# faircloth-lab/tapir

Hardware: AMD Instinct MI355X
Metric: alignment columns/sec (site-rate+PI) (higher is better)
Workload: dtype f64

## Files before the change

tapir_amd/csrc/launch_constants.hpp:

```cpp
#pragma once
#include <cstddef>
#include <cstdint>

namespace tphip {

constexpr int kFirstStepMinTaxa = 32;
constexpr int kSiteBlock = 64;
constexpr int kReserveShift = 16;
constexpr int kShareWeightShift = 10;
constexpr double kDefaultReserve = 0.15;
constexpr int kTailFillsBig = 5, kTailFillsMid = 3, kTailFillsSmall = 2;
constexpr double kTailFracBig = 0.4, kTailFracMid = 0.3;
constexpr int kMixedLoci = 8;
constexpr int kMixedLdsHeader = kMixedLoci * 64 + 64 + 32;
constexpr int kMixedColBits = 28;
constexpr int kSiteLdsHeader = 160;
constexpr int kStreamWords = -1;
constexpr int kStreamWordsSpill = -2;
constexpr int kMixedVariant = 100;

#ifndef TPHIP_LIK_BLOCK
#define TPHIP_LIK_BLOCK 128
#endif
constexpr int kLikBlock = TPHIP_LIK_BLOCK;
constexpr int kGradBlock = 128;
constexpr int kGradWaves = kGradBlock / 64;
constexpr int kGradEF = 12;
constexpr int kGradSlots = 4;
constexpr size_t kValueWorkspaceBytes = (size_t)1 << 30;
constexpr int kValueTipRow = 20;
constexpr int kValueMaxDepth = 5;
constexpr int kGrad2Block = 128;
constexpr int kGrad2Waves = kGrad2Block / 64;
constexpr int kGrad2EF = 12;
constexpr int kGrad2MaxRDepth = 8;

constexpr int kPiBlock = 256;
constexpr int kPiColsPerThread = 4;
constexpr int kPiChunk = kPiBlock * kPiColsPerThread;

enum : int32_t { DEDUP_AUTO = 0, DEDUP_OFF = 1, DEDUP_ON = 2 };
constexpr int64_t kDedupAutoMinColumns = 1 << 20;

}
```

tapir_amd/csrc/pi_kernels.hpp:

```cpp
#pragma once
#include <hip/hip_runtime.h>
#include <cstdint>
#include "gtr_model.hpp"
#include "tree_program.hpp"
#include "quadpack_device.hpp"
#include "site_rate_params.hpp"
#include "pi_rate.hpp"
#include "tphip.h"
#include "wave_sum.hpp"

namespace tphip {

constexpr int kTimeTile = 16;
constexpr int kIvTile = 8;

struct ClassifyParams {
    const uint8_t* states;
    int64_t ncols_total;
    int32_t ntaxa;
    const LocusModel* models;
    const int64_t* locus_offsets;
    const int32_t* chunk_locus;
    const int32_t* chunk_index;
    double* rate;
    double* subst;
    double* lnl;
    uint8_t* flag;
    int32_t* nres;
    double chrono_length;
    const int2* steps;
    int32_t tail_pops;
    int32_t max_pops;
    uint32_t* packed;
    double start_scale;
    uint64_t* hash;
};

typedef const __attribute__((address_space(4))) int2 ConstInt2;
__device__ __forceinline__ ConstInt2* as_constant(const int2* p) { return (ConstInt2*)(uintptr_t)p; }

struct ColumnScan {
    unsigned uni = 0;
    int resolved = 0, informative = 0;
    unsigned changes = 0;
    int base[3] = {0, 0, 0};
};

struct ColumnScan4 {
    static constexpr uint32_t k01 = 0x01010101u, k0f = 0x0f0f0f0fu;
    uint32_t uni4 = 0, set4 = k0f;
    uint32_t res8 = 0, inf8 = 0, chg8 = 0;
    uint32_t a8 = 0, c8 = 0, g8 = 0;
    int base[3][4] = {{0, 0, 0, 0}, {0, 0, 0, 0}, {0, 0, 0, 0}};
    uint64_t hsh[4] = {0x243F6A8885A308D3ull, 0x243F6A8885A308D3ull, 0x243F6A8885A308D3ull, 0x243F6A8885A308D3ull};
    int resolved[4] = {0, 0, 0, 0}, informative[4] = {0, 0, 0, 0};
    unsigned changes[4] = {0, 0, 0, 0};
    unsigned long long stk[4] = {0, 0, 0, 0};
    static __device__ __forceinline__ uint32_t nonzero(uint32_t x) { return ((x + k0f) >> 4) & k01; }
    static __device__ __forceinline__ uint32_t is15(uint32_t x) { return ((x + k01) >> 4) & k01; }
    static __device__ __forceinline__ uint32_t spread(uint32_t b) {
        uint32_t s = b << 4;
        asm("" : "+v"(s));
        return s - b;
    }
    __device__ __forceinline__ void flush() {
#pragma unroll
        for (int j = 0; j < 4; ++j) {
            resolved[j] += (int)((res8 >> (8 * j)) & 0xffu);
            informative[j] += (int)((inf8 >> (8 * j)) & 0xffu);
            changes[j] += (chg8 >> (8 * j)) & 0xffu;
            base[0][j] += (int)((a8 >> (8 * j)) & 0xffu);
            base[1][j] += (int)((c8 >> (8 * j)) & 0xffu);
            base[2][j] += (int)((g8 >> (8 * j)) & 0xffu);
        }
        res8 = inf8 = chg8 = 0;
        a8 = c8 = g8 = 0;
    }
    __device__ __forceinline__ void fitch_join(uint32_t x4) {
        const uint32_t both = set4 & x4;
        const uint32_t empty = nonzero(both) ^ k01;
        chg8 += empty;
        set4 = both | ((set4 | x4) & spread(empty));
    }
    __device__ __forceinline__ void fitch_push() {
#pragma unroll
        for (int j = 0; j < 4; ++j) stk[j] = (stk[j] << 4) | ((set4 >> (8 * j)) & 15u);
        set4 = k0f;
    }
    __device__ __forceinline__ void fitch_pop() {
        uint32_t x4 = 0;
#pragma unroll
        for (int j = 0; j < 4; ++j) { x4 |= (uint32_t)(stk[j] & 15ull) << (8 * j); stk[j] >>= 4; }
        fitch_join(x4);
    }
    __device__ __forceinline__ uint32_t tip(uint32_t v) {
        uint32_t m4 = v & k0f;
        m4 |= spread(nonzero(m4) ^ k01);
        const uint32_t res = is15(m4) ^ k01;
        uni4 |= m4 & spread(res);
        res8 += res;
        const uint32_t single = nonzero(m4 & (m4 - k01)) ^ k01;
        inf8 += single;
        a8 += single & m4;
        c8 += single & (m4 >> 1);
        g8 += single & (m4 >> 2);
        fitch_join(m4);
        return m4;
    }
    static __device__ __forceinline__ void pack8(const uint32_t* m, uint32_t* word) {
        const uint32_t a01 = m[0] | (m[1] << 4), a23 = m[2] | (m[3] << 4), a45 = m[4] | (m[5] << 4), a67 = m[6] | (m[7] << 4);
        const uint32_t t_lo = __builtin_amdgcn_perm(a23, a01, 0x05010400u);
        const uint32_t t_hi = __builtin_amdgcn_perm(a23, a01, 0x07030602u);
        const uint32_t u_lo = __builtin_amdgcn_perm(a67, a45, 0x05010400u);
        const uint32_t u_hi = __builtin_amdgcn_perm(a67, a45, 0x07030602u);
        word[0] = __builtin_amdgcn_perm(u_lo, t_lo, 0x05040100u);
        word[1] = __builtin_amdgcn_perm(u_lo, t_lo, 0x07060302u);
        word[2] = __builtin_amdgcn_perm(u_hi, t_hi, 0x05040100u);
        word[3] = __builtin_amdgcn_perm(u_hi, t_hi, 0x07060302u);
    }
    __device__ __forceinline__ ColumnScan column(int j) const {
        ColumnScan c;
        c.uni = (uni4 >> (8 * j)) & 15u;
        c.resolved = resolved[j];
        c.informative = informative[j];
        c.changes = changes[j];
        c.base[0] = base[0][j]; c.base[1] = base[1][j]; c.base[2] = base[2][j];
// ... 112 lines not shown
            for (int j = 0; j < 4; ++j) {
                uint64_t h = (c.hsh[j] ^ word[j]) * 0x9E3779B97F4A7C15ull;
                c.hsh[j] = h ^ (h >> 29);
            }
        }
    };
    const int ngroups = (P.ntaxa + 7) >> 3;
    uint32_t b0[8], b1[8];
    load_group(0, b0);
    int g = 0;
    for (; g + 1 < ngroups; g += 2) {
        load_group(g + 1, b1);
        asm volatile("" ::: "memory");
        group(g, b0);
        if (g + 2 < ngroups) load_group(g + 2, b0);
        asm volatile("" ::: "memory");
        group(g + 1, b1);
    }
    if (g < ngroups) group(g, b0);
    for (int q = P.tail_pops; q > 0; --q) c.fitch_pop();
}

__global__ __launch_bounds__(kPiBlock) void classify_kernel(ClassifyParams P) {
    const int locus = P.chunk_locus[blockIdx.x];
    const int64_t lo = P.locus_offsets[locus], hi = P.locus_offsets[locus + 1];
    const LocusModel* __restrict__ M = P.models + locus;
    const int64_t c0 = lo + (int64_t)P.chunk_index[blockIdx.x] * kPiChunk + 4 * (int64_t)threadIdx.x;
    if (c0 >= hi) return;
    const bool full = (c0 + 4 <= hi);
    const bool aligned = full && ((reinterpret_cast<uintptr_t>(P.states) & 3u) == 0) && ((P.ncols_total & 3) == 0) &&
                         ((c0 & 3) == 0);
    const int n = full ? 4 : (int)(hi - c0);
    const bool fast = __all(aligned);
    ColumnScan4 c;
    if (fast) {
        if (P.max_pops <= kMaxUnrolledPops) classify_scan<true, true>(P, c0, n, c);
        else classify_scan<true, false>(P, c0, n, c);
    } else {
        classify_scan<false, false>(P, c0, n, c);
    }
    c.flush();
    uint8_t f[4] = {0, 0, 0, 0};
    double ex[4];
    exit_rates(M, ex);
#pragma unroll
    for (int j = 0; j < 4; ++j) if (j < n) classify_finish(P, M, c0 + j, c.column(j), ex, f[j]);
    if (P.hash) {
#pragma unroll
        for (int j = 0; j < 4; ++j) if (j < n) P.hash[c0 + j] = c.hsh[j] ^ (c.hsh[j] >> 32);
    }
    if (fast) {
        *reinterpret_cast<int4*>(P.nres + c0) = make_int4(c.informative[0], c.informative[1], c.informative[2], c.informative[3]);
        *reinterpret_cast<uint32_t*>(P.flag + c0) = (uint32_t)f[0] | ((uint32_t)f[1] << 8) | ((uint32_t)f[2] << 16) | ((uint32_t)f[3] << 24);
    } else {
#pragma unroll
        for (int j = 0; j < 4; ++j) {
            if (j < n) { P.nres[c0 + j] = c.informative[j]; P.flag[c0 + j] = f[j]; }
        }
    }
}

template <int kCompactBlock>
__global__ __launch_bounds__(kCompactBlock) void compact_kernel(const uint8_t* __restrict__ flag, const int64_t* __restrict__ locus_offsets,
                                                                int32_t* __restrict__ work_cols, int32_t* __restrict__ work_count) {
    constexpr int kWaves = kCompactBlock / 64;
    __shared__ int wave_tot[kWaves];
    __shared__ int running;
// ... 436 lines not shown
        double r[kPiColsPerThread];
        bool ok[kPiColsPerThread];
        pi_pack_chunk(P, base, hi, packed_rate, r, ok);
#pragma unroll
        for (int j = 0; j < kPiColsPerThread; ++j) n_ok += ok[j] ? 1 : 0;
    }
    double* out = P.partial + (size_t)chunk * (P.T + 2 * P.n_i);
    for (int k0 = 0; k0 < P.n_i; k0 += kIvSplitTile) {
        int a[kIvSplitTile], b[kIvSplitTile];
#pragma unroll
        for (int kk = 0; kk < kIvSplitTile; ++kk) {
            const int k = (k0 + kk < P.n_i) ? k0 + kk : P.n_i - 1;
            a[kk] = __builtin_amdgcn_readfirstlane(P.intervals[2 * k]);
            b[kk] = __builtin_amdgcn_readfirstlane(P.intervals[2 * k + 1]);
        }
        double si[kIvSplitTile], se[kIvSplitTile];
#pragma unroll
        for (int kk = 0; kk < kIvSplitTile; ++kk) { si[kk] = 0.0; se[kk] = 0.0; }
#pragma unroll 1
        for (int j = 0; j < n_ok; ++j) {
            const double rj = packed_rate[j * kPiBlock + (int)threadIdx.x];
            GkFactors F;
            double have_h = -1.0;
#pragma unroll
            for (int kk = 0; kk < kIvSplitTile; ++kk) {
                if (k0 + kk < P.n_i) {
                    int ai = a[kk], bi = b[kk];
                    asm volatile("" : "+s"(ai), "+s"(bi));
                    const double aj = (double)ai, bj = (double)bi;
                    double res, err = 0.0;
                    if (P.integ_mode == TPHIP_INTEG_QUADPACK) {
                        const double hl = 0.5 * (bj - aj);
                        if (4.0 * rj * hl < 30.0) {
                            if (hl != have_h) { gk_factors(rj, hl, F); have_h = hl; }
                            quad_townsend_factored(aj, bj, rj, F, res, err);
                        } else {
                            const QuadResult g = quad_townsend_generic(aj, bj, rj);
                            res = g.result;
                            err = g.abserr;
                        }
                    } else {
                        res = integral_closed(aj, bj, rj);
                    }
                    si[kk] += res;
                    se[kk] += err;
                }
            }
        }
#pragma unroll
        for (int kk = 0; kk < kIvSplitTile; ++kk) {
            if (k0 + kk < P.n_i) {
                const double s1 = wave_sum(si[kk]), s2 = wave_sum(se[kk]);
                if (lane == 0) { red[2 * kk][wave] = s1; red[2 * kk + 1][wave] = s2; }
            }
        }
        __syncthreads();
        if (threadIdx.x < 2 * kIvSplitTile && k0 + (int)(threadIdx.x >> 1) < P.n_i) {
            const int kk = threadIdx.x >> 1, which = threadIdx.x & 1;
            out[P.T + which * P.n_i + k0 + kk] =
                ((red[threadIdx.x][0] + red[threadIdx.x][1]) + red[threadIdx.x][2]) + red[threadIdx.x][3];
        }
        __syncthreads();
    }
}

constexpr int kPiReduceBlock = 64;
__global__ __launch_bounds__(kPiReduceBlock) void pi_reduce_kernel(const double* __restrict__ partial, const int64_t* __restrict__ locus_chunk_offsets,
                                 int32_t T, const int32_t* __restrict__ times, int32_t n_t, int32_t n_i,
// ... 82 lines not shown
```

tapir_amd/csrc/quadpack_device.hpp:

```cpp
#pragma once
#include <hip/hip_runtime.h>
#include <cfloat>
#include "fast_exp.hpp"

namespace tphip {

template <bool TAB>
__device__ __forceinline__ double townsend_pi(double t, double r, const double* __restrict__ etab) {
#pragma clang fp contract(off)
    const double x = -(4.0 * r * t);
    if constexpr (TAB) return 16.0 * (r * r) * t * exp_nonpos_tab(fmin(x, 0.0), etab);
    else return 16.0 * (r * r) * t * exp(x);
}

struct GK21 {
    double result, abserr, resabs, resasc;
};

__device__ __constant__ const double kXgk[11] = {
    0.995657163025808080735527280689003, 0.973906528517171720077964012084452, 0.930157491355708226001207180059508,
    0.865063366688984510732096688423493, 0.780817726586416897063717578345042, 0.679409568299024406234327365114874,
    0.562757134668604683339000099272694, 0.433395394129247190799265943165784, 0.294392862701460198131126603103866,
    0.148874338981631210884826001129720, 0.0};
__device__ __constant__ const double kWgk[11] = {
    0.011694638867371874278064396062192, 0.032558162307964727478818972459390, 0.054755896574351996031381300244580,
    0.075039674810919952767043140916190, 0.093125454583697605535065465083366, 0.109387158802297641899210590325805,
    0.123491976262065851077958109585166, 0.134709217311473325928054001771707, 0.142775938577060080797094273138717,
    0.147739104901338491374841515972068, 0.149445554002916905664936468389821};
__device__ __constant__ const double kWg[5] = {
    0.066671344308688137593568809893332, 0.149451349150580593145776339657697, 0.219086362515982043995534934228163,
    0.269266719309996355091226921569469, 0.295524224714752870173815619188769};

template <bool TAB>
__device__ __forceinline__ GK21 dqk21(double rate, double a, double b, const double* __restrict__ etab) {
#pragma clang fp contract(off)
    const double epmach = DBL_EPSILON, uflow = DBL_MIN;
    double fv1[10], fv2[10];
    const double centr = 0.5 * (a + b), hlgth = 0.5 * (b - a), dhlgth = fabs(hlgth);
    double resg = 0.0;
    const double fc = townsend_pi<TAB>(centr, rate, etab);
    double resk = kWgk[10] * fc;
    double resabs = fabs(resk);
#pragma unroll
    for (int j = 0; j < 5; ++j) {
        const int jtw = 2 * j + 1;
        const double absc = hlgth * kXgk[jtw];
        const double f1 = townsend_pi<TAB>(centr - absc, rate, etab), f2 = townsend_pi<TAB>(centr + absc, rate, etab);
        fv1[jtw] = f1; fv2[jtw] = f2;
        const double fsum = f1 + f2;
        resg += kWg[j] * fsum;
        resk += kWgk[jtw] * fsum;
        resabs += kWgk[jtw] * (fabs(f1) + fabs(f2));
    }
#pragma unroll
    for (int j = 0; j < 5; ++j) {
        const int jtwm1 = 2 * j;
        const double absc = hlgth * kXgk[jtwm1];
        const double f1 = townsend_pi<TAB>(centr - absc, rate, etab), f2 = townsend_pi<TAB>(centr + absc, rate, etab);
        fv1[jtwm1] = f1; fv2[jtwm1] = f2;
        const double fsum = f1 + f2;
        resk += kWgk[jtwm1] * fsum;
        resabs += kWgk[jtwm1] * (fabs(f1) + fabs(f2));
    }
    const double reskh = resk * 0.5;
    double resasc = kWgk[10] * fabs(fc - reskh);
#pragma unroll
    for (int j = 0; j < 10; ++j) resasc += kWgk[j] * (fabs(fv1[j] - reskh) + fabs(fv2[j] - reskh));
    GK21 o;
    o.result = resk * hlgth;
    o.resabs = resabs * dhlgth;
    o.resasc = resasc * dhlgth;
    double abserr = fabs((resk - resg) * hlgth);
    if (o.resasc != 0.0 && abserr != 0.0) {
        const double q = 200.0 * abserr / o.resasc;
        const double q15 = q * sqrt(q);
        abserr = o.resasc * fmin(1.0, q15);
    }
    if (o.resabs > uflow / (50.0 * epmach)) abserr = fmax((epmach * 50.0) * o.resabs, abserr);
    o.abserr = abserr;
    return o;
}

struct GkFactors {
    double fm[10];
    double fp[10];
};

__device__ __forceinline__ void gk_factors(double rate, double hlgth, GkFactors& F) {
#pragma clang fp contract(off)
#pragma unroll
    for (int j = 0; j < 10; ++j) {
        const double absc = hlgth * kXgk[j];
        F.fm[j] = exp(-(4.0 * rate * absc));
        F.fp[j] = 1.0 / F.fm[j];
    }
}

__device__ __forceinline__ GK21 dqk21_factored(double rate, double a, double b, const GkFactors& F) {
#pragma clang fp contract(off)
    const double epmach = DBL_EPSILON, uflow = DBL_MIN;
    double fv1[10], fv2[10];
    const double centr = 0.5 * (a + b), hlgth = 0.5 * (b - a), dhlgth = fabs(hlgth);
    const double c16 = 16.0 * (rate * rate);
    const double ec = exp(-(4.0 * rate * centr));
    double resg = 0.0;
    const double fc = c16 * centr * ec;
    double resk = kWgk[10] * fc;
    double resabs = fabs(resk);
#pragma unroll
    for (int j = 0; j < 5; ++j) {
        const int jtw = 2 * j + 1;
        const double absc = hlgth * kXgk[jtw];
        const double f1 = c16 * (centr - absc) * (ec * F.fp[jtw]), f2 = c16 * (centr + absc) * (ec * F.fm[jtw]);
        fv1[jtw] = f1; fv2[jtw] = f2;
        const double fsum = f1 + f2;
        resg += kWg[j] * fsum;
        resk += kWgk[jtw] * fsum;
        resabs += kWgk[jtw] * (fabs(f1) + fabs(f2));
    }
#pragma unroll
    for (int j = 0; j < 5; ++j) {
        const int jtwm1 = 2 * j;
        const double absc = hlgth * kXgk[jtwm1];
        const double f1 = c16 * (centr - absc) * (ec * F.fp[jtwm1]), f2 = c16 * (centr + absc) * (ec * F.fm[jtwm1]);
        fv1[jtwm1] = f1; fv2[jtwm1] = f2;
        const double fsum = f1 + f2;
        resk += kWgk[jtwm1] * fsum;
        resabs += kWgk[jtwm1] * (fabs(f1) + fabs(f2));
    }
    const double reskh = resk * 0.5;
    double resasc = kWgk[10] * fabs(fc - reskh);
#pragma unroll
    for (int j = 0; j < 10; ++j) resasc += kWgk[j] * (fabs(fv1[j] - reskh) + fabs(fv2[j] - reskh));
    GK21 o;
    o.result = resk * hlgth;
    o.resabs = resabs * dhlgth;
    o.resasc = resasc * dhlgth;
    double abserr = fabs((resk - resg) * hlgth);
    if (o.resasc != 0.0 && abserr != 0.0) {
        const double q = 200.0 * abserr / o.resasc;
        const double q15 = q * sqrt(q);
        abserr = o.resasc * fmin(1.0, q15);
    }
    if (o.resabs > uflow / (50.0 * epmach)) abserr = fmax((epmach * 50.0) * o.resabs, abserr);
    o.abserr = abserr;
    return o;
}

__device__ inline void dqpsrt(int limit, int last, int* maxerr, double* ermax, const double* elist, int* iord, int* nrmax) {
    if (last <= 2) {
        iord[1] = 1; iord[2] = 2;
    } else {
        const double errmax = elist[*maxerr];
        if (*nrmax != 1) {
            const int ido = *nrmax - 1;
            for (int i = 1; i <= ido; ++i) {
                const int isucc = iord[*nrmax - 1];
                if (errmax <= elist[isucc]) break;
                iord[*nrmax] = isucc;
                --*nrmax;
            }
        }
        int jupbn = last;
        if (last > (limit / 2 + 2)) jupbn = limit + 3 - last;
        const double errmin = elist[last];
        const int jbnd = jupbn - 1;
// ... 195 lines not shown
            if (ierro == 3) abserr += correc;
            if (ier == 0) ier = 3;
            if (result != 0.0 && area != 0.0) {
                if (abserr / fabs(result) > errsum / fabs(area)) sum_lists = true;
            } else if (abserr > errsum) {
                sum_lists = true;
            }
        }
        (void)ksgn;
    }
    if (sum_lists) {
        result = 0.0;
        for (int k = 1; k <= last; ++k) result += rlist[k];
        abserr = errsum;
    }
    *result_out = result;
    *abserr_out = abserr;
}

template <bool TAB>
__device__ __forceinline__ void quad_townsend(double a, double b, double rate, const double* __restrict__ etab, double& result,
                                              double& abserr) {
#pragma clang fp contract(off)
    const double epsabs = 1.49e-8, epsrel = 1.49e-8, epmach = DBL_EPSILON;
    const GK21 g = dqk21<TAB>(rate, a, b, etab);
    result = g.result;
    abserr = g.abserr;
    const double errbnd = fmax(epsabs, epsrel * fabs(g.result));
    const bool roundoff = (g.abserr <= 100.0 * epmach * g.resabs && g.abserr > errbnd);
    const bool accept = roundoff || (g.abserr <= errbnd && g.abserr != g.resasc) || g.abserr == 0.0;
    if (!accept) dqagse_adaptive<TAB>(rate, a, b, g, etab, &result, &abserr);
}

__device__ __forceinline__ void quad_townsend_factored(double a, double b, double rate, const GkFactors& F, double& result,
                                                       double& abserr) {
#pragma clang fp contract(off)
    const double epsabs = 1.49e-8, epsrel = 1.49e-8, epmach = DBL_EPSILON;
    const GK21 g = dqk21_factored(rate, a, b, F);
    result = g.result;
    abserr = g.abserr;
    const double errbnd = fmax(epsabs, epsrel * fabs(g.result));
    const bool roundoff = (g.abserr <= 100.0 * epmach * g.resabs && g.abserr > errbnd);
    const bool accept = roundoff || (g.abserr <= errbnd && g.abserr != g.resasc) || g.abserr == 0.0;
    if (!accept) dqagse_adaptive<false>(rate, a, b, g, nullptr, &result, &abserr);
}

__device__ __forceinline__ double integral_closed(double a, double b, double r) {
    const double xa = 4.0 * r * a, d = 4.0 * r * (b - a);
    double m = 0.0, g = 0.0;
    if (d < 0.1) {
        double term = d;
        for (int k = 1; k < 40; ++k) {
            const double add = term * (double)(k - 1);
            m += (k & 1) ? term : -term;
            g += (k & 1) ? -add : add;
            if (k > 1 && add <= 1e-20 * fabs(g)) break;
            term = term * d / (double)(k + 1);
        }
    } else {
        const double e = exp(-d);
        m = 1.0 - e;
        g = m - d * e;
    }
    return exp(-xa) * (xa * m + g);
}

}
```

tapir_amd/csrc/site_driver.hip:

```cpp
#include <hip/hip_runtime.h>

#include <cstdio>
#include <cstdlib>

#include "dedup_kernels.hpp"
#include "pi_kernels.hpp"
#include "tphip_internal.hpp"

extern "C" {

int tphip_profile_enable(tphip_plan* p, int32_t on) {
    if (!p) return fail(TPHIP_ERR_INVALID, "null plan");
    HIP_TRY(hipSetDevice(p->device));
    if (on && p->ev.empty()) {
        p->ev.resize(4 * kProfileRing);
        for (auto& e : p->ev) HIP_TRY(hipEventCreate(&e));
    }
    p->profile = on != 0;
    return TPHIP_OK;
}

static int profile_drain(tphip_plan* p) {
    for (int s = 0; s < p->ev_used; ++s) {
        float ms = 0;
// ... 29 lines not shown
        for (tphip_plan* q : p->parts) {
            HIP_TRY(hipMemcpy(&w, q->d_evals.p + which, sizeof w, hipMemcpyDeviceToHost));
            v += w;
        }
    } else {
        HIP_TRY(hipMemcpy(&v, p->d_evals.p + which, sizeof v, hipMemcpyDeviceToHost));
    }
    *out = (int64_t)v;
    return TPHIP_OK;
}

int tphip_last_eval_count(tphip_plan* p, int64_t* evals) {
    const int rc = last_count(p, 0, evals);
    if (rc == TPHIP_OK && !p->last_run_in_parts && getenv("TPHIP_SITE_TRACE_ROUNDS")) {
        unsigned long long c[8];
        HIP_TRY(hipMemcpy(c, p->d_evals.p, sizeof c, hipMemcpyDeviceToHost));
        if (c[5]) fprintf(stderr, "site_rate_kernel: %llu waves with work, evaluations %llu, rounds mean %.1f max %llu (lane use %.1f %%), wave time mean %.1f us max %.1f us\n",
                          c[5], c[0], (double)c[1] / c[5], c[2], 100.0 * c[0] / (64.0 * c[1]), 0.01 * c[3] / c[5], 0.01 * c[4]);
    }
    return rc;
}

int tphip_last_round_count(tphip_plan* p, int64_t* rounds) { return last_count(p, 1, rounds); }


static ClassifyParams classify_params(const tphip_plan* p, const uint8_t* d_states, double* rate, double* subst, double* lnl, uint8_t* flag,
                                      int32_t* nres, uint32_t* packed, uint64_t* hash, double start_scale) {
    ClassifyParams C{};
    C.states = d_states; C.ncols_total = p->ncols; C.ntaxa = p->ntaxa; C.models = p->d_models.p;
    C.locus_offsets = p->d_offsets.p; C.chunk_locus = p->d_pi_chunk_locus.p; C.chunk_index = p->d_pi_chunk_index.p;
    C.rate = rate; C.subst = subst; C.lnl = lnl; C.flag = flag; C.nres = nres;
    C.chrono_length = p->prog.chrono_length;
    C.steps = (const int2*)p->d_cls_steps.p; C.tail_pops = p->prog.cls_tail_pops; C.max_pops = p->prog.cls_max_pops;
    C.packed = packed; C.start_scale = start_scale; C.hash = hash;
    return C;
}

static DedupParams dedup_params(const tphip_plan* p, const ClassifyParams& C, int32_t* dup_of, unsigned long long* tab_key,
                                int32_t* tab_val, int32_t* on, int32_t mode, bool results) {
    DedupParams D{};
    D.locus_offsets = p->d_offsets.p; D.chunk_locus = p->d_pi_chunk_locus.p; D.chunk_index = p->d_pi_chunk_index.p;
    D.hash = C.hash; D.packed = C.packed; D.nwords = p->nwords; D.ncols_total = p->ncols; D.flag = C.flag;
    D.dup_of = dup_of; D.tab_key = tab_key; D.tab_val = tab_val; D.on = on; D.mode = mode;
    if (results) { D.rate = C.rate; D.subst = C.subst; D.lnl = C.lnl; }
    return D;
}

static void launch_compact_chunked(tphip_plan* p, const uint8_t* d_flag, const double* d_lnl, int32_t* work_cols, int32_t* work_count,
                                  int32_t* work_class, void* ws, hipStream_t st) {
    int2* cnt = (int2*)((char*)ws + p->ws.chunk_cnt);
    const dim3 chunks((unsigned)p->n_pi_chunks), loci((unsigned)p->nloci), block(kCompactChunkBlock);
    if (work_class) {
        compact_count_kernel<true><<<chunks, block, 0, st>>>(d_flag, d_lnl, p->d_offsets.p, p->d_pi_chunk_locus.p, p->d_pi_chunk_index.p, cnt);
        compact_scan_kernel<true><<<loci, block, 0, st>>>(p->d_locus_pichunk_offsets.p, cnt, work_count, work_class);
        compact_scatter_kernel<true><<<chunks, block, 0, st>>>(d_flag, d_lnl, p->d_offsets.p, p->d_pi_chunk_locus.p, p->d_pi_chunk_index.p, cnt,
                                                               work_count, work_class, p->site.reserve_q, work_cols);
    } else {
        compact_count_kernel<false><<<chunks, block, 0, st>>>(d_flag, nullptr, p->d_offsets.p, p->d_pi_chunk_locus.p, p->d_pi_chunk_index.p, cnt);
        compact_scan_kernel<false><<<loci, block, 0, st>>>(p->d_locus_pichunk_offsets.p, cnt, work_count, nullptr);
        compact_scatter_kernel<false><<<chunks, block, 0, st>>>(d_flag, nullptr, p->d_offsets.p, p->d_pi_chunk_locus.p, p->d_pi_chunk_index.p, cnt,
                                                                work_count, nullptr, 0, work_cols);
    }
}

int launch_site_rates(tphip_plan* p, const uint8_t* d_states, double* d_rate, double* d_subst, double* d_lnl,
                      uint8_t* d_flag, int32_t* d_nres, void* ws, hipStream_t st, int slot) {
    p->last_run_in_parts = false;
    const auto at = [ws](size_t offset) { return (void*)((char*)ws + offset); };
    int32_t* work_cols = (int32_t*)at(p->ws.work_cols);
    int32_t* work_count = (int32_t*)at(p->ws.work_count);
    int64_t* work_prefix = (int64_t*)at(p->ws.work_prefix);
    int64_t* slice_prefix = (int64_t*)at(p->ws.slice_prefix);
    const bool dedup = p->site.dedup_mode != DEDUP_OFF && p->n_pi_chunks > 0;
    const ClassifyParams C = classify_params(p, d_states, d_rate, d_subst, d_lnl, d_flag, d_nres, (uint32_t*)at(p->ws.packed),
                                             dedup ? (uint64_t*)at(p->ws.hash) : nullptr,
                                             (p->site.start_rule == TPHIP_START_REFERENCE) ? 0.0 : 1.0);
    DedupParams D{};
    if (dedup) D = dedup_params(p, C, (int32_t*)at(p->ws.dup_of), (unsigned long long*)at(p->ws.tab_key), (int32_t*)at(p->ws.tab_val),
                                (int32_t*)at(p->ws.dedup_on), p->site.dedup_mode, true);
    if (p->n_pi_chunks > 0) {
        classify_kernel<<<dim3((unsigned)p->n_pi_chunks), dim3(kPiBlock), 0, st>>>(C);
        if (dedup) {
            if (p->max_locus_cols > 2048) dedup_estimate_kernel<1024><<<dim3((unsigned)p->nloci), dim3(1024), 0, st>>>(D);
            else dedup_estimate_kernel<256><<<dim3((unsigned)p->nloci), dim3(256), 0, st>>>(D);
            dedup_insert_kernel<<<dim3((unsigned)p->n_pi_chunks), dim3(256), 0, st>>>(D);
            dedup_resolve_kernel<<<dim3((unsigned)p->n_pi_chunks), dim3(256), 0, st>>>(D);
        }
        if (p->site.share_work) {
            int32_t* work_class = (int32_t*)at(p->ws.work_class);
            if (p->site.compact_chunked) {
                launch_compact_chunked(p, d_flag, d_lnl, work_cols, work_count, work_class, ws, st);
            } else {
                int32_t* scratch = p->site.reserve_q > 0 ? (int32_t*)at(p->ws.work_cols2) : nullptr;
                if (p->max_locus_cols > 2048) compact_classes_kernel<1024><<<dim3((unsigned)p->nloci), dim3(1024), 0, st>>>(d_flag, p->d_offsets.p, work_cols, work_count, d_lnl, p->site.reserve_q, scratch, work_class);
                else compact_classes_kernel<256><<<dim3((unsigned)p->nloci), dim3(256), 0, st>>>(d_flag, p->d_offsets.p, work_cols, work_count, d_lnl, p->site.reserve_q, scratch, work_class);
            }
            ScanClasses SC;
            SC.cls = work_class; SC.reserve_q = p->site.reserve_q; SC.w_slow = p->site.w_slow; SC.w_easy = p->site.w_easy;
            SC.locus_offsets = p->d_offsets.p;
            SC.wprefix = (int64_t*)at(p->ws.work_wprefix); SC.part_prefix = (int64_t*)at(p->ws.part_prefix);
            SC.part_start = (int64_t*)at(p->ws.part_start);
            HIP_TRY(launch_scan_counts_kernel(st, work_count, p->nloci, p->site.chunk_cols, work_prefix, slice_prefix, &SC));
        } else {
            if (p->site.compact_chunked) launch_compact_chunked(p, d_flag, nullptr, work_cols, work_count, nullptr, ws, st);
            else if (p->max_locus_cols > 2048) compact_kernel<1024><<<dim3((unsigned)p->nloci), dim3(1024), 0, st>>>(d_flag, p->d_offsets.p, work_cols, work_count);
            else compact_kernel<256><<<dim3((unsigned)p->nloci), dim3(256), 0, st>>>(d_flag, p->d_offsets.p, work_cols, work_count);
            HIP_TRY(launch_scan_counts_kernel(st, work_count, p->nloci, p->site.chunk_cols, work_prefix, slice_prefix, nullptr));
        }
    }
    HIP_TRY(hipMemsetAsync(p->d_evals.p, 0, 8 * sizeof(unsigned long long), st));
    const SiteKernelArgs A = site_kernel_args(p->site, p->nwords, p->prog.stack_depth, p->n_site_chunks);
    SiteParams S = plan_site_params(p, d_states, true);
    S.packed = C.packed; S.nwords = p->nwords;
    S.work_cols = work_cols; S.work_count = work_count;
// ... 11 lines not shown
    if (slot >= 0) HIP_TRY(hipEventRecord(p->ev[4 * slot + 0], st));
    if (p->n_site_chunks > 0)
        HIP_TRY(launch_site_rate_kernel(A.variant, p->model, dim3((unsigned)A.grid), A.lds_bytes, st, S));
    if (slot >= 0) HIP_TRY(hipEventRecord(p->ev[4 * slot + 1], st));
    if (dedup) dedup_scatter_kernel<<<dim3((unsigned)p->n_pi_chunks), dim3(256), 0, st>>>(D);
    HIP_TRY(hipGetLastError());
    return TPHIP_OK;
}

__global__ __launch_bounds__(256) void eb_start_scale_kernel(const int64_t* __restrict__ locus_offsets, const uint8_t* __restrict__ flag,
                                                            const double* __restrict__ start_log, double chrono_length,
                                                            double* __restrict__ start) {
    __shared__ double red[256];
    const int locus = blockIdx.x;
    const int64_t lo = locus_offsets[locus], hi = locus_offsets[locus + 1];
    double sum = 0.0;
    for (int64_t c = lo + threadIdx.x; c < hi; c += 256)
        if (flag[c] == TPHIP_FLAG_OK) sum += exp(start_log[c]);
    red[threadIdx.x] = sum;
    __syncthreads();
    for (int o = 128; o > 0; o >>= 1) {
        if ((int)threadIdx.x < o) red[threadIdx.x] += red[threadIdx.x + o];
        __syncthreads();
    }
    if (threadIdx.x == 0) start[locus] = (red[0] > 0.0 && hi > lo) ? red[0] / (double)(hi - lo) : 1.0 / chrono_length;
}

int tphip_internal_eb_prepare(tphip_plan* p, const uint8_t* d_states, const EbPrep* B, int32_t use_patterns, double* d_start,
                              void* stream) {
    hipStream_t st = (hipStream_t)stream;
    if (p->n_pi_chunks <= 0) return TPHIP_OK;
    const ClassifyParams C = classify_params(p, d_states, B->scratch[0], B->scratch[1], B->scratch[2], B->flag, B->nres, B->packed,
                                             use_patterns ? B->hash : nullptr, 1.0);
    classify_kernel<<<dim3((unsigned)p->n_pi_chunks), dim3(kPiBlock), 0, st>>>(C);
    if (d_start)
        eb_start_scale_kernel<<<dim3((unsigned)p->nloci), dim3(256), 0, st>>>(p->d_offsets.p, B->flag, B->scratch[0],
                                                                             p->prog.chrono_length, d_start);
    HIP_TRY(hipMemsetAsync(B->flag, TPHIP_FLAG_OK, (size_t)p->ncols, st));
    HIP_TRY(hipMemsetAsync(B->dup_of, 0xff, sizeof(int32_t) * (size_t)p->ncols, st));
    if (use_patterns) {
        const DedupParams D = dedup_params(p, C, B->dup_of, B->tab_key, B->tab_val, B->on, DEDUP_ON, false);
        if (p->max_locus_cols > 2048) dedup_estimate_kernel<1024><<<dim3((unsigned)p->nloci), dim3(1024), 0, st>>>(D);
        else dedup_estimate_kernel<256><<<dim3((unsigned)p->nloci), dim3(256), 0, st>>>(D);
        dedup_insert_kernel<<<dim3((unsigned)p->n_pi_chunks), dim3(256), 0, st>>>(D);
        dedup_resolve_kernel<<<dim3((unsigned)p->n_pi_chunks), dim3(256), 0, st>>>(D);
        if (p->max_locus_cols > 2048) compact_kernel<1024><<<dim3((unsigned)p->nloci), dim3(1024), 0, st>>>(B->flag, p->d_offsets.p, B->work_cols, B->work_count);
        else compact_kernel<256><<<dim3((unsigned)p->nloci), dim3(256), 0, st>>>(B->flag, p->d_offsets.p, B->work_cols, B->work_count);
    }
    HIP_TRY(hipGetLastError());
    return TPHIP_OK;
}

int launch_pi_tables(tphip_plan* p, const double* d_rates, const int32_t* d_nres, double* d_tables, void* ws, hipStream_t st,
                     int slot) {
    PiParams Q = plan_pi_params(p, d_rates, d_nres);
    Q.partial = (double*)((char*)ws + p->ws.partial);
    if (slot >= 0) HIP_TRY(hipEventRecord(p->ev[4 * slot + 2], st));
    if (p->n_pi_chunks > 0) {
        const dim3 grid((unsigned)p->n_pi_chunks), block(kPiBlock);
        if (p->site.pi_split) {
            pi_net_kernel<<<grid, block, 0, st>>>(Q);
            if (p->n_i > 0) pi_interval_kernel<<<grid, block, 0, st>>>(Q);
        } else {
            pi_partial_kernel<<<grid, block, 0, st>>>(Q);
        }
    }
    pi_reduce_kernel<<<dim3((unsigned)p->nloci), dim3(kPiReduceBlock), 0, st>>>(Q.partial, p->d_locus_pichunk_offsets.p, p->T,
// ... 209 lines not shown
```

tapir_amd/csrc/tphip.hip:

```cpp
#include <hip/hip_runtime.h>

#include <algorithm>
#include <cmath>
#include <cstddef>
#include <cstdlib>
#include <cstring>
#include <string>
#include <vector>

#include "gtr_setup_kernel.hpp"
#include "tphip_internal.hpp"

using namespace tphip;

thread_local std::string g_tphip_err;

static void free_host_buffers(struct tphip_plan* p);
static void free_parts(struct tphip_plan* p);

extern "C" {

int tphip_version(void) { return TPHIP_VERSION; }

const char* tphip_last_error(void) { return g_tphip_err.c_str(); }
// ... 275 lines not shown
        if (d->locus_offsets[l + 1] < d->locus_offsets[l]) return fail(TPHIP_ERR_INVALID, "locus_offsets not monotone");
        if (const int rc = check_locus_model(d->pi, d->exch, l)) return rc;
    }
    const int64_t ncols = d->locus_offsets[d->nloci];
    if (ncols >= (int64_t)1 << 31) return fail(TPHIP_ERR_INVALID, "more than 2^31-1 columns in one batch");
    std::vector<double> cat;
    if (d->ncat > 1) {
        if (d->ncat > 16) return fail(TPHIP_ERR_INVALID, "at most 16 rate categories");
        if (!d->cat_rate || !d->cat_weight) return fail(TPHIP_ERR_INVALID, "rate categories need cat_rate and cat_weight");
        double wsum = 0;
        for (int k = 0; k < d->ncat; ++k) {
            if (!(d->cat_rate[k] > 0.0) || !(d->cat_weight[k] > 0.0) || !std::isfinite(d->cat_rate[k]) || !std::isfinite(d->cat_weight[k]))
                return fail(TPHIP_ERR_INVALID, "category rates and weights must be positive and finite");
            wsum += d->cat_weight[k];
        }
        cat.resize(2 * (size_t)d->ncat);
        for (int k = 0; k < d->ncat; ++k) { cat[k] = d->cat_rate[k]; cat[d->ncat + k] = std::log(d->cat_weight[k] / wsum); }
    }
    const PlanKnobs knobs = knobs_from_env();

    tphip_plan* p = new tphip_plan();
    p->device = d->device; p->ntaxa = d->ntaxa; p->nnodes = d->nnodes; p->nloci = d->nloci; p->ncols = ncols;
    p->T = d->T; p->n_t = d->n_t; p->n_i = d->n_i; p->integ_mode = d->integ_mode;
    p->threshold = d->threshold; p->round_decimals = d->round_decimals; p->correction = d->correction;
    p->model = d->model;
    p->ncat = cat.empty() ? 0 : d->ncat;
    std::string terr = build_tree_program(d->ntaxa, d->nnodes, d->parent, d->branch_len, d->leaf_taxon, &p->prog);
    if (!terr.empty()) { delete p; return fail(TPHIP_ERR_INVALID, "tree: " + terr); }
    if (p->prog.nleaves != d->ntaxa) {
        delete p;
        return fail(TPHIP_ERR_INVALID, "tree: the number of leaves differs from the number of alignment rows");
    }
    if (site_lds_bytes(p->prog.stack_depth) > 160 * 1024) { delete p; return fail(TPHIP_ERR_INVALID, "tree needs a deeper LDS stack than 160 KiB allows"); }
    int64_t ntips = 0;
    for (const TreeOp& op : p->prog.ops) ntips += op.code <= OP_TIP_MUL;
    p->nwords = (int32_t)((ntips + 7) / 8);
    p->h_offsets.assign(d->locus_offsets, d->locus_offsets + d->nloci + 1);
    for (int64_t l = 0; l < d->nloci; ++l)
        p->max_locus_cols = std::max<int64_t>(p->max_locus_cols, d->locus_offsets[l + 1] - d->locus_offsets[l]);

    hipError_t e = hipSetDevice(d->device);
    if (e != hipSuccess) return plan_setup_failed(p, e);
    hipDeviceProp_t prop;
    if (hipGetDeviceProperties(&prop, d->device) != hipSuccess) { tphip_plan_destroy(p); return fail(TPHIP_ERR_HIP, "hipGetDeviceProperties failed"); }
    p->num_cus = prop.multiProcessorCount;
    SiteShape shape;
    shape.ncols = ncols; shape.nloci = d->nloci; shape.max_locus_cols = p->max_locus_cols; shape.ntaxa = d->ntaxa;
    shape.nwords = p->nwords; shape.stack_depth = p->prog.stack_depth; shape.model = d->model; shape.ncat = d->ncat;
    shape.start_rule = d->start_rule; shape.pattern_dedup = d->pattern_dedup; shape.T = d->T; shape.n_i = d->n_i;
    p->site = decide_site_launch(shape, p->num_cus, knobs, [&](int variant, size_t lds_bytes) {
        int per_cu = 0;
        return site_rate_kernel_occupancy(variant, shape.model, lds_bytes, &per_cu) == hipSuccess ? per_cu : 0;
    });
    p->host_split = host_split_groups(knobs);

    const ChunkTables chunks = build_chunk_tables(p->h_offsets.data(), d->nloci, p->site.chunk_cols);
    p->n_site_chunks = (int64_t)chunks.site_chunk_locus.size();
    p->n_pi_chunks = (int64_t)chunks.pi_chunk_locus.size();
    p->ws = layout_workspace(shape, p->site, p->n_pi_chunks);

    e = upload_plan(p, d, cat, chunks);
    if (e != hipSuccess) return plan_setup_failed(p, e);

    configure_locus_launch(p, knobs);
    p->saved = save_desc(d);
    *out = p;
// ... 267 lines not shown
```

tapir_amd/csrc/tree_program.hpp:

```cpp
#pragma once
#include <algorithm>
#include <cstdint>
#include <string>
#include <vector>

namespace tphip {

enum : int32_t { OP_TIP_SET = 0, OP_TIP_MUL = 1, OP_BRANCH = 2, OP_PUSH = 3, OP_POP_MUL = 4,
                 OP_CHERRY = 5 };
enum : int32_t { OP_CODE_MASK = 0xff,
                 OP_PUSH_BEFORE = 0x100,
                 OP_POP_AFTER = 0x200 };

struct TreeOp {
    int32_t code;
    int32_t taxon;
    double t;
};
static_assert(sizeof(TreeOp) == 16, "TreeOp is read with one s_load_dwordx4");

struct TreeProgram {
    std::vector<TreeOp> ops;
    std::vector<TreeOp> fused_ops;
    std::vector<int32_t> op_node;
    std::vector<int32_t> op_tape;
    std::vector<int32_t> op_partner;
    int32_t ntape = 0;
    std::vector<int32_t> cls_steps;
    int32_t cls_tail_pops = 0;
    int32_t cls_max_pops = 0;
    int32_t stack_depth = 0;
    double chrono_length = 0;
    int32_t nleaves = 0;
};

inline std::string build_tree_program(int32_t ntaxa, int32_t nnodes, const int32_t* parent, const double* blen,
                                      const int32_t* leaf_taxon, TreeProgram* out) {
    if (nnodes < 3) return "tree needs at least two leaves";
    std::vector<std::vector<int32_t>> kids(nnodes);
    int32_t root = -1;
    for (int32_t n = 0; n < nnodes; ++n) {
        int32_t p = parent[n];
        if (p < 0) {
            if (root >= 0) return "tree has more than one root";
            root = n;
        } else {
            if (p >= nnodes || p <= n) return "tree nodes must be in post-order (parent index > child index)";
            kids[p].push_back(n);
        }
    }
    if (root != nnodes - 1) return "root must be the last node";
    std::vector<char> seen(ntaxa > 0 ? ntaxa : 0, 0);
    out->chrono_length = 0;
    out->nleaves = 0;
    for (int32_t n = 0; n < nnodes; ++n) {
        bool leaf = kids[n].empty();
        if (leaf) {
            int32_t tx = leaf_taxon[n];
            if (tx < 0 || tx >= ntaxa) return "leaf_taxon out of range";
            if (seen[tx]) return "two leaves map to the same alignment row";
            seen[tx] = 1;
            ++out->nleaves;
        } else if (leaf_taxon[n] >= 0) {
// ... 37 lines not shown
                if (!first) { out->ops.push_back({OP_PUSH, 0, 0.0}); out->op_node.push_back(-1); }
                st.push_back({c, 0});
            }
        } else {
            st.pop_back();
            if (!st.empty()) {
                out->ops.push_back({OP_BRANCH, 0, blen[n]});
                out->op_node.push_back(n);
                bool was_first = (st.back().next == 1);
                if (!was_first) { out->ops.push_back({OP_POP_MUL, 0, 0.0}); out->op_node.push_back(-1); }
            }
        }
    }
    out->op_tape.assign(out->ops.size(), -1);
    out->op_partner.assign(out->ops.size(), -1);
    out->ntape = 0;
    std::vector<int32_t> pushed;
    for (size_t i = 0; i < out->ops.size(); ++i) {
        const int32_t code = out->ops[i].code;
        if (code == OP_BRANCH) {
            out->op_tape[i] = out->ntape++;
        } else if (code == OP_PUSH) {
            out->op_tape[i] = out->ntape++;
            pushed.push_back(out->op_tape[i]);
        } else if (code == OP_POP_MUL) {
            if (pushed.empty()) return "internal error: POP_MUL without PUSH";
            out->op_partner[i] = pushed.back();
            pushed.pop_back();
        }
    }
    if (!pushed.empty()) return "internal error: unbalanced PUSH";
    out->cls_steps.clear();
    out->cls_max_pops = 0;
    int32_t pops = 0, push = 0;
    for (const TreeOp& op : out->ops) {
        if (op.code == OP_PUSH) {
            if (push) return "internal error: two PUSH ops between tips";
            push = 1;
        } else if (op.code == OP_POP_MUL) {
            if (push) return "internal error: POP_MUL after a PUSH between tips";
            ++pops;
        } else if (op.code == OP_TIP_SET || op.code == OP_TIP_MUL) {
            out->cls_steps.push_back(op.taxon);
            out->cls_steps.push_back(pops * 2 + push);
            out->cls_max_pops = std::max(out->cls_max_pops, pops);
            pops = push = 0;
        }
    }
    if (push) return "internal error: PUSH after the last tip";
    out->cls_tail_pops = pops;
    while (out->cls_steps.size() % 16) {
        out->cls_steps.push_back(out->cls_steps[out->cls_steps.size() - 2]);
        out->cls_steps.push_back(0);
    }
    out->fused_ops.clear();
    int32_t pending = 0;
    for (size_t i = 0; i < out->ops.size(); ++i) {
        const TreeOp& a = out->ops[i];
        const bool has_next = i + 1 < out->ops.size();
        if (a.code == OP_PUSH && has_next && out->ops[i + 1].code == OP_TIP_SET) {
            pending = OP_PUSH_BEFORE;
        } else if (a.code == OP_TIP_SET && has_next && out->ops[i + 1].code == OP_TIP_MUL && out->ops[i + 1].t == a.t) {
            out->fused_ops.push_back({OP_CHERRY | pending, a.taxon, a.t});
            pending = 0;
            ++i;
        } else if (a.code == OP_BRANCH && has_next && out->ops[i + 1].code == OP_POP_MUL) {
            out->fused_ops.push_back({OP_BRANCH | OP_POP_AFTER, a.taxon, a.t});
            ++i;
        } else {
            out->fused_ops.push_back({a.code | pending, a.taxon, a.t});
            pending = 0;
        }
    }
    return "";
}

}
```

Measured before the change: 809.4 million.

## Move Fitch parsimony stack to LDS and load quadrature tables via scalar constant path

The per-thread Fitch stack in the classify kernel was four 64-bit shift registers holding 4-bit sets. It is replaced with an LDS-resident stack of packed 32-bit words plus a register-held top, with the depth computed on the host. This removes the 16-level depth cap and the per-push/pop shift-and-mask work, at the cost of LDS traffic and dynamic shared-memory allocation that may reduce occupancy. Separately, the Gauss-Kronrod tables in the factored quadrature path are read through an address_space(4) pointer forced into scalar registers, so they load via scalar constant loads rather than vector loads.

```diff
diff --git a/tapir_amd/csrc/launch_constants.hpp b/tapir_amd/csrc/launch_constants.hpp
--- a/tapir_amd/csrc/launch_constants.hpp
+++ b/tapir_amd/csrc/launch_constants.hpp
@@ -38,6 +38,8 @@
 constexpr int kPiBlock = 256;
 constexpr int kPiColsPerThread = 4;
 constexpr int kPiChunk = kPiBlock * kPiColsPerThread;
+constexpr size_t classify_lds_bytes(int32_t depth) { return (size_t)depth * kPiBlock * sizeof(uint32_t); }
+constexpr size_t kClassifyMaxLdsBytes = 64 * 1024;
 
 enum : int32_t { DEDUP_AUTO = 0, DEDUP_OFF = 1, DEDUP_ON = 2 };
 constexpr int64_t kDedupAutoMinColumns = 1 << 20;
diff --git a/tapir_amd/csrc/pi_kernels.hpp b/tapir_amd/csrc/pi_kernels.hpp
--- a/tapir_amd/csrc/pi_kernels.hpp
+++ b/tapir_amd/csrc/pi_kernels.hpp
@@ -31,6 +31,7 @@
     const int2* steps;
     int32_t tail_pops;
     int32_t max_pops;
+    int32_t depth;
     uint32_t* packed;
     double start_scale;
     uint64_t* hash;
@@ -55,7 +56,9 @@
     uint64_t hsh[4] = {0x243F6A8885A308D3ull, 0x243F6A8885A308D3ull, 0x243F6A8885A308D3ull, 0x243F6A8885A308D3ull};
     int resolved[4] = {0, 0, 0, 0}, informative[4] = {0, 0, 0, 0};
     unsigned changes[4] = {0, 0, 0, 0};
-    unsigned long long stk[4] = {0, 0, 0, 0};
+    uint32_t top = k0f;
+    uint32_t* stack;
+    __device__ __forceinline__ explicit ColumnScan4(uint32_t* stack_end) : stack(stack_end) {}
     static __device__ __forceinline__ uint32_t nonzero(uint32_t x) { return ((x + k0f) >> 4) & k01; }
     static __device__ __forceinline__ uint32_t is15(uint32_t x) { return ((x + k01) >> 4) & k01; }
     static __device__ __forceinline__ uint32_t spread(uint32_t b) {
@@ -83,15 +86,15 @@
         set4 = both | ((set4 | x4) & spread(empty));
     }
     __device__ __forceinline__ void fitch_push() {
-#pragma unroll
-        for (int j = 0; j < 4; ++j) stk[j] = (stk[j] << 4) | ((set4 >> (8 * j)) & 15u);
+        stack -= kPiBlock;
+        *stack = top;
+        top = set4;
         set4 = k0f;
     }
     __device__ __forceinline__ void fitch_pop() {
-        uint32_t x4 = 0;
-#pragma unroll
-        for (int j = 0; j < 4; ++j) { x4 |= (uint32_t)(stk[j] & 15ull) << (8 * j); stk[j] >>= 4; }
-        fitch_join(x4);
+        fitch_join(top);
+        top = *stack;
+        stack += kPiBlock;
     }
     __device__ __forceinline__ uint32_t tip(uint32_t v) {
         uint32_t m4 = v & k0f;
@@ -270,7 +273,8 @@
                          ((c0 & 3) == 0);
     const int n = full ? 4 : (int)(hi - c0);
     const bool fast = __all(aligned);
-    ColumnScan4 c;
+    extern __shared__ uint32_t fitch_stack[];
+    ColumnScan4 c(fitch_stack + P.depth * kPiBlock + threadIdx.x);
     if (fast) {
         if (P.max_pops <= kMaxUnrolledPops) classify_scan<true, true>(P, c0, n, c);
         else classify_scan<true, false>(P, c0, n, c);
@@ -773,8 +777,8 @@
                     if (P.integ_mode == TPHIP_INTEG_QUADPACK) {
                         const double hl = 0.5 * (bj - aj);
                         if (4.0 * rj * hl < 30.0) {
-                            if (hl != have_h) { gk_factors(rj, hl, F); have_h = hl; }
-                            quad_townsend_factored(aj, bj, rj, F, res, err);
+                            if (hl != have_h) { gk_factors<true>(rj, hl, F); have_h = hl; }
+                            quad_townsend_factored<true>(aj, bj, rj, F, res, err);
                         } else {
                             const QuadResult g = quad_townsend_generic(aj, bj, rj);
                             res = g.result;
diff --git a/tapir_amd/csrc/quadpack_device.hpp b/tapir_amd/csrc/quadpack_device.hpp
--- a/tapir_amd/csrc/quadpack_device.hpp
+++ b/tapir_amd/csrc/quadpack_device.hpp
@@ -1,6 +1,7 @@
 #pragma once
 #include <hip/hip_runtime.h>
 #include <cfloat>
+#include <cstdint>
 #include "fast_exp.hpp"
 
 namespace tphip {
@@ -31,6 +32,18 @@
     0.066671344308688137593568809893332, 0.149451349150580593145776339657697, 0.219086362515982043995534934228163,
     0.269266719309996355091226921569469, 0.295524224714752870173815619188769};
 
+typedef const __attribute__((address_space(4))) double ConstDouble;
+template <bool kLoaded>
+__device__ __forceinline__ auto gk_table(const double* tab) {
+    if constexpr (kLoaded) {
+        uintptr_t p = (uintptr_t)tab;
+        asm volatile("" : "+s"(p));
+        return (ConstDouble*)p;
+    } else {
+        return tab;
+    }
+}
+
 template <bool TAB>
 __device__ __forceinline__ GK21 dqk21(double rate, double a, double b, const double* __restrict__ etab) {
 #pragma clang fp contract(off)
@@ -86,52 +99,56 @@
     double fp[10];
 };
 
+template <bool kLoaded = false>
 __device__ __forceinline__ void gk_factors(double rate, double hlgth, GkFactors& F) {
 #pragma clang fp contract(off)
+    const auto xgk = gk_table<kLoaded>(kXgk);
 #pragma unroll
     for (int j = 0; j < 10; ++j) {
-        const double absc = hlgth * kXgk[j];
+        const double absc = hlgth * xgk[j];
         F.fm[j] = exp(-(4.0 * rate * absc));
         F.fp[j] = 1.0 / F.fm[j];
     }
 }
 
+template <bool kLoaded = false>
 __device__ __forceinline__ GK21 dqk21_factored(double rate, double a, double b, const GkFactors& F) {
 #pragma clang fp contract(off)
     const double epmach = DBL_EPSILON, uflow = DBL_MIN;
+    const auto xgk = gk_table<kLoaded>(kXgk), wgk = gk_table<kLoaded>(kWgk), wg = gk_table<kLoaded>(kWg);
     double fv1[10], fv2[10];
     const double centr = 0.5 * (a + b), hlgth = 0.5 * (b - a), dhlgth = fabs(hlgth);
     const double c16 = 16.0 * (rate * rate);
     const double ec = exp(-(4.0 * rate * centr));
     double resg = 0.0;
     const double fc = c16 * centr * ec;
-    double resk = kWgk[10] * fc;
+    double resk = wgk[10] * fc;
     double resabs = fabs(resk);
 #pragma unroll
     for (int j = 0; j < 5; ++j) {
         const int jtw = 2 * j + 1;
-        const double absc = hlgth * kXgk[jtw];
+        const double absc = hlgth * xgk[jtw];
         const double f1 = c16 * (centr - absc) * (ec * F.fp[jtw]), f2 = c16 * (centr + absc) * (ec * F.fm[jtw]);
         fv1[jtw] = f1; fv2[jtw] = f2;
         const double fsum = f1 + f2;
-        resg += kWg[j] * fsum;
-        resk += kWgk[jtw] * fsum;
-        resabs += kWgk[jtw] * (fabs(f1) + fabs(f2));
+        resg += wg[j] * fsum;
+        resk += wgk[jtw] * fsum;
+        resabs += wgk[jtw] * (fabs(f1) + fabs(f2));
     }
 #pragma unroll
     for (int j = 0; j < 5; ++j) {
         const int jtwm1 = 2 * j;
-        const double absc = hlgth * kXgk[jtwm1];
+        const double absc = hlgth * xgk[jtwm1];
         const double f1 = c16 * (centr - absc) * (ec * F.fp[jtwm1]), f2 = c16 * (centr + absc) * (ec * F.fm[jtwm1]);
         fv1[jtwm1] = f1; fv2[jtwm1] = f2;
         const double fsum = f1 + f2;
-        resk += kWgk[jtwm1] * fsum;
-        resabs += kWgk[jtwm1] * (fabs(f1) + fabs(f2));
+        resk += wgk[jtwm1] * fsum;
+        resabs += wgk[jtwm1] * (fabs(f1) + fabs(f2));
     }
     const double reskh = resk * 0.5;
-    double resasc = kWgk[10] * fabs(fc - reskh);
-#pragma unroll
-    for (int j = 0; j < 10; ++j) resasc += kWgk[j] * (fabs(fv1[j] - reskh) + fabs(fv2[j] - reskh));
+    double resasc = wgk[10] * fabs(fc - reskh);
+#pragma unroll
+    for (int j = 0; j < 10; ++j) resasc += wgk[j] * (fabs(fv1[j] - reskh) + fabs(fv2[j] - reskh));
     GK21 o;
     o.result = resk * hlgth;
     o.resabs = resabs * dhlgth;
@@ -393,11 +410,12 @@
     if (!accept) dqagse_adaptive<TAB>(rate, a, b, g, etab, &result, &abserr);
 }
 
+template <bool kLoaded = false>
 __device__ __forceinline__ void quad_townsend_factored(double a, double b, double rate, const GkFactors& F, double& result,
                                                        double& abserr) {
 #pragma clang fp contract(off)
     const double epsabs = 1.49e-8, epsrel = 1.49e-8, epmach = DBL_EPSILON;
-    const GK21 g = dqk21_factored(rate, a, b, F);
+    const GK21 g = dqk21_factored<kLoaded>(rate, a, b, F);
     result = g.result;
     abserr = g.abserr;
     const double errbnd = fmax(epsabs, epsrel * fabs(g.result));
diff --git a/tapir_amd/csrc/site_driver.hip b/tapir_amd/csrc/site_driver.hip
--- a/tapir_amd/csrc/site_driver.hip
+++ b/tapir_amd/csrc/site_driver.hip
@@ -85,8 +85,13 @@
     C.rate = rate; C.subst = subst; C.lnl = lnl; C.flag = flag; C.nres = nres;
     C.chrono_length = p->prog.chrono_length;
     C.steps = (const int2*)p->d_cls_steps.p; C.tail_pops = p->prog.cls_tail_pops; C.max_pops = p->prog.cls_max_pops;
+    C.depth = p->prog.cls_depth;
     C.packed = packed; C.start_scale = start_scale; C.hash = hash;
     return C;
+}
+
+static void launch_classify(const tphip_plan* p, const ClassifyParams& C, hipStream_t st) {
+    classify_kernel<<<dim3((unsigned)p->n_pi_chunks), dim3(kPiBlock), classify_lds_bytes(C.depth), st>>>(C);
 }
 
 static DedupParams dedup_params(const tphip_plan* p, const ClassifyParams& C, int32_t* dup_of, unsigned long long* tab_key,
@@ -132,7 +137,7 @@
     if (dedup) D = dedup_params(p, C, (int32_t*)at(p->ws.dup_of), (unsigned long long*)at(p->ws.tab_key), (int32_t*)at(p->ws.tab_val),
                                 (int32_t*)at(p->ws.dedup_on), p->site.dedup_mode, true);
     if (p->n_pi_chunks > 0) {
-        classify_kernel<<<dim3((unsigned)p->n_pi_chunks), dim3(kPiBlock), 0, st>>>(C);
+        launch_classify(p, C, st);
         if (dedup) {
             if (p->max_locus_cols > 2048) dedup_estimate_kernel<1024><<<dim3((unsigned)p->nloci), dim3(1024), 0, st>>>(D);
             else dedup_estimate_kernel<256><<<dim3((unsigned)p->nloci), dim3(256), 0, st>>>(D);
@@ -210,7 +215,7 @@
     if (p->n_pi_chunks <= 0) return TPHIP_OK;
     const ClassifyParams C = classify_params(p, d_states, B->scratch[0], B->scratch[1], B->scratch[2], B->flag, B->nres, B->packed,
                                              use_patterns ? B->hash : nullptr, 1.0);
-    classify_kernel<<<dim3((unsigned)p->n_pi_chunks), dim3(kPiBlock), 0, st>>>(C);
+    launch_classify(p, C, st);
     if (d_start)
         eb_start_scale_kernel<<<dim3((unsigned)p->nloci), dim3(256), 0, st>>>(p->d_offsets.p, B->flag, B->scratch[0],
                                                                              p->prog.chrono_length, d_start);
diff --git a/tapir_amd/csrc/tphip.hip b/tapir_amd/csrc/tphip.hip
--- a/tapir_amd/csrc/tphip.hip
+++ b/tapir_amd/csrc/tphip.hip
@@ -331,6 +331,7 @@
         return fail(TPHIP_ERR_INVALID, "tree: the number of leaves differs from the number of alignment rows");
     }
     if (site_lds_bytes(p->prog.stack_depth) > 160 * 1024) { delete p; return fail(TPHIP_ERR_INVALID, "tree needs a deeper LDS stack than 160 KiB allows"); }
+    if (classify_lds_bytes(p->prog.cls_depth) > kClassifyMaxLdsBytes) { delete p; return fail(TPHIP_ERR_INVALID, "tree needs a deeper parsimony stack than 64 KiB of LDS allow"); }
     int64_t ntips = 0;
     for (const TreeOp& op : p->prog.ops) ntips += op.code <= OP_TIP_MUL;
     p->nwords = (int32_t)((ntips + 7) / 8);
diff --git a/tapir_amd/csrc/tree_program.hpp b/tapir_amd/csrc/tree_program.hpp
--- a/tapir_amd/csrc/tree_program.hpp
+++ b/tapir_amd/csrc/tree_program.hpp
@@ -29,6 +29,7 @@
     std::vector<int32_t> cls_steps;
     int32_t cls_tail_pops = 0;
     int32_t cls_max_pops = 0;
+    int32_t cls_depth = 0;
     int32_t stack_depth = 0;
     double chrono_length = 0;
     int32_t nleaves = 0;
@@ -132,7 +133,8 @@
     if (!pushed.empty()) return "internal error: unbalanced PUSH";
     out->cls_steps.clear();
     out->cls_max_pops = 0;
-    int32_t pops = 0, push = 0;
+    out->cls_depth = 0;
+    int32_t pops = 0, push = 0, parked = 0;
     for (const TreeOp& op : out->ops) {
         if (op.code == OP_PUSH) {
             if (push) return "internal error: two PUSH ops between tips";
@@ -144,11 +146,16 @@
             out->cls_steps.push_back(op.taxon);
             out->cls_steps.push_back(pops * 2 + push);
             out->cls_max_pops = std::max(out->cls_max_pops, pops);
+            parked -= pops;
+            if (parked < 0) return "internal error: POP_MUL on an empty stack";
+            parked += push;
+            out->cls_depth = std::max(out->cls_depth, parked);
             pops = push = 0;
         }
     }
     if (push) return "internal error: PUSH after the last tip";
     out->cls_tail_pops = pops;
+    if (parked != pops) return "internal error: parked sets left after the last tip";
     while (out->cls_steps.size() % 16) {
         out->cls_steps.push_back(out->cls_steps[out->cls_steps.size() - 2]);
         out->cls_steps.push_back(0);
```

After: 814.2 million, median of 6. No clear change (+0.6%).
